# zju3dv/pvnet

Hardware: NVIDIA H100
Metric: images/sec (480x640, K=9) backbone+vote (higher is better)
Workload: dtype tf32 (fp32 storage, fp32 accumulate; vote fp32/fp64)

## Files before the change

pvnet_b200/csrc/conv_tc.cu:

```cuda
#include "conv_tc.cuh"
#include "ptx.cuh"

#include <cstdlib>
#include <mutex>
#include <new>

namespace pvnet {

struct ConvGeom {
    int Ho, Wo;
    int tiles_x, tiles_y, total_m_tiles;
    int TH, TW;
    int taps, cin_chunks, cin_pad;
    int Cout, BN;
    int out_cs, out_co;
    int res_cs, res_co;
    int act;
    int round_out;
    signed char tap_map[9];
    short tap_ox[9], tap_oy[9];
    int n_items;
    int stages;
};

struct AMaps {
    CUtensorMap m[4];
};

constexpr int CONV_THREADS = 288;
constexpr int CONV_KC = 32;
constexpr int CONV_A_BYTES = 128 * CONV_KC * 4;
constexpr int CONV_SLAB = 32;
constexpr int CONV_SLAB_BYTES = 128 * CONV_SLAB * 4;
constexpr int CONV_EPI_BAR = 1;

template <int BN, bool MC>
__global__ void __launch_bounds__(CONV_THREADS, 1)
    k_conv_tap(const __grid_constant__ AMaps amaps, const __grid_constant__ CUtensorMap tmB,
               const __grid_constant__ CUtensorMap tmOut, const __grid_constant__ CUtensorMap tmRes,
               const __grid_constant__ ConvGeom g, const float *__restrict__ bias, const int has_res)
{
    constexpr int B_BYTES = BN * CONV_KC * 4;
    constexpr int STAGE_BYTES = CONV_A_BYTES + B_BYTES;
    constexpr int SLABS = BN / CONV_SLAB;
    const int STAGES = g.stages;
    extern __shared__ uint8_t smem_raw[];
    uint8_t *smem = reinterpret_cast<uint8_t *>((reinterpret_cast<uintptr_t>(smem_raw) + 1023) & ~uintptr_t(1023));
    uint8_t *slab = smem + (size_t)STAGES * STAGE_BYTES;
    uint64_t *full = reinterpret_cast<uint64_t *>(slab + 2 * CONV_SLAB_BYTES);
    uint64_t *empty = full + STAGES;
    uint64_t *res_full = empty + STAGES;
    uint64_t *res_free = res_full + 2;

    const int warp = threadIdx.x >> 5, lane = threadIdx.x & 31;
    const int tiles_per_img = g.tiles_x * g.tiles_y;
    const int n_tiles_n = g.Cout / BN;
    const int nkb = g.taps * g.cin_chunks;
    const uint32_t crank = MC ? ptx::cluster_ctarank() : 0u;
    const int unit = MC ? (int)blockIdx.x >> 1 : (int)blockIdx.x, nunits = MC ? (int)gridDim.x >> 1 : (int)gridDim.x;
    auto item_tile = [&](int item, int &m_tile, int &n0) {
        const int mi = item / n_tiles_n;
        n0 = (item - mi * n_tiles_n) * BN;
        m_tile = MC ? min(2 * mi + (int)crank, g.total_m_tiles - 1) : mi;
    };

    if (threadIdx.x == 0) {
        for (int s = 0; s < STAGES; ++s) {
            ptx::mbar_init(&full[s], 1);
            ptx::mbar_init(&empty[s], MC ? 16 : 8);
        }
        for (int i = 0; i < 2; ++i) {
            ptx::mbar_init(&res_full[i], 1);
            ptx::mbar_init(&res_free[i], 1);
        }
        ptx::fence_barrier_init();
    }
    __syncthreads();
    if (MC) ptx::cluster_sync();

    if (warp == 8) {
        if (lane == 0) {
            int r_item = has_res ? unit : g.n_items, r_slab = 0;
            uint32_t rq = 0;
            auto poll_res = [&]() {
                if (r_item >= g.n_items) return;
                const uint32_t b = rq & 1u;
                if (!ptx::mbar_test_wait(&res_free[b], ((rq >> 1) & 1u) ^ 1u)) return;
                int m_tile, n0;
                item_tile(r_item, m_tile, n0);
                const int img = m_tile / tiles_per_img;
                const int trem = m_tile - img * tiles_per_img;
                const int tyi = trem / g.tiles_x, txi = trem - tyi * g.tiles_x;
                ptx::mbar_arrive_expect_tx(&res_full[b], (uint32_t)CONV_SLAB_BYTES);
                ptx::tma_load_4d(slab + b * CONV_SLAB_BYTES, &tmRes, &res_full[b], n0 + r_slab * CONV_SLAB, txi * g.TW,
                                 tyi * g.TH, img);
                ++rq;
                if (++r_slab == SLABS) {
                    r_slab = 0;
                    r_item += nunits;
                }
            };
            int s = 0;
            uint32_t ph = 0;
            for (int item = unit; item < g.n_items; item += nunits) {
                int m_tile, n0;
                item_tile(item, m_tile, n0);
                const int img = m_tile / tiles_per_img;
                const int trem = m_tile - img * tiles_per_img;
                const int tyi = trem / g.tiles_x, txi = trem - tyi * g.tiles_x;
                const int y0 = tyi * g.TH, x0 = txi * g.TW;
                for (int tap = 0; tap < g.taps; ++tap)
                    for (int cc = 0; cc < g.cin_chunks; ++cc) {
                        poll_res();
                        while (!(has_res ? ptx::mbar_test_wait(&empty[s], ph ^ 1u) : ptx::mbar_try_wait(&empty[s], ph ^ 1u)))
                            poll_res();
                        ptx::mbar_arrive_expect_tx(&full[s], (uint32_t)STAGE_BYTES);
                        uint8_t *sa = smem + (size_t)s * STAGE_BYTES;
                        ptx::tma_load_4d(sa, &amaps.m[g.tap_map[tap]], &full[s], cc * CONV_KC, x0 + g.tap_ox[tap],
                                         y0 + g.tap_oy[tap], img);
                        if (MC)
                            ptx::tma_load_2d_mc(sa + CONV_A_BYTES + crank * (B_BYTES / 2), &tmB, &full[s],
                                                tap * g.cin_pad + cc * CONV_KC, n0 + (int)crank * (BN / 2), (uint16_t)0x3);
                        else
                            ptx::tma_load_2d(sa + CONV_A_BYTES, &tmB, &full[s], tap * g.cin_pad + cc * CONV_KC, n0);
                        if (++s == STAGES) {
                            s = 0;
                            ph ^= 1u;
                        }
                    }
            }
            while (r_item < g.n_items) poll_res();
        }
    } else {
        const int wg = warp >> 2, wq = warp & 3;
        const int g8 = lane >> 2, t4 = lane & 3;
        const uint32_t smem_u = ptx::smem_u32(smem);
        auto release = [&](int st) {
            ptx::mbar_arrive(&empty[st]);
            if (MC) ptx::mbar_arrive_cluster(&empty[st], crank ^ 1u);
        };
        int s = 0;
        uint32_t ph = 0, sq = 0;
        for (int item = unit; item < g.n_items; item += nunits) {
            float acc[BN / 2];
#pragma unroll
            for (int i = 0; i < BN / 2; ++i) acc[i] = 0.f;
            int prev = -1;
            for (int kb = 0; kb < nkb; ++kb) {
                ptx::mbar_wait(&full[s], ph);
                const uint32_t sa = smem_u + (uint32_t)s * (uint32_t)STAGE_BYTES;
                const uint64_t adesc = ptx::make_kmajor_desc(sa + (uint32_t)(wg * 64 * 128), 128);
                const uint64_t bdesc = ptx::make_kmajor_desc(sa + (uint32_t)CONV_A_BYTES, 128);
                ptx::wgmma_fence();
#pragma unroll
                for (int k = 0; k < CONV_KC / 8; ++k)
                    ptx::Wgmma<BN>::ss(acc, adesc + (uint64_t)(2 * k), bdesc + (uint64_t)(2 * k), (kb | k) != 0 ? 1u : 0u);
                ptx::wgmma_commit();
                ptx::wgmma_wait<1>();
                ptx::fence_regs(acc);
                if (prev >= 0 && lane == 0) release(prev);
                prev = s;
                if (++s == STAGES) {
                    s = 0;
                    ph ^= 1u;
                }
            }
            ptx::wgmma_wait<0>();
            ptx::fence_regs(acc);
            if (lane == 0) release(prev);

            int m_tile, n0;
            item_tile(item, m_tile, n0);
            const int img = m_tile / tiles_per_img;
            const int trem = m_tile - img * tiles_per_img;
            const int tyi = trem / g.tiles_x, txi = trem - tyi * g.tiles_x;
            const uint32_t row_off = (uint32_t)((wg * 64 + wq * 16 + g8) * 128 + (t4 & 1) * 8);
            const uint32_t swz = (uint32_t)(((t4 >> 1) ^ g8) << 4);
            const uint32_t slab_u = ptx::smem_u32(slab);
#pragma unroll
            for (int j = 0; j < SLABS; ++j, ++sq) {
                const uint32_t b = sq & 1u;
                const uint32_t base = slab_u + b * (uint32_t)CONV_SLAB_BYTES + row_off;
                float2 bv[4];
#pragma unroll
                for (int jj = 0; jj < 4; ++jj)
                    bv[jj] = __ldg(reinterpret_cast<const float2 *>(bias + n0 + CONV_SLAB * j + 8 * jj + 2 * t4));
                if (has_res) ptx::mbar_wait(&res_full[b], (sq >> 1) & 1u);
                else ptx::named_bar_sync(CONV_EPI_BAR, 256);
#pragma unroll
                for (int jj = 0; jj < 4; ++jj)
#pragma unroll
                    for (int h = 0; h < 2; ++h) {
                        const uint32_t addr = base + (uint32_t)(h * 8 * 128) + (swz ^ (uint32_t)(32 * jj));
                        const int a = 4 * (4 * j + jj) + 2 * h;
                        float2 v = make_float2(acc[a] + bv[jj].x, acc[a + 1] + bv[jj].y);
                        if (has_res) {
                            const float2 r = ptx::lds64(addr);
                            v.x += r.x;
                            v.y += r.y;
                        }
                        v.x = epi_act(v.x, g.act, g.round_out);
                        v.y = epi_act(v.y, g.act, g.round_out);
                        ptx::sts64(addr, v);
                    }
                ptx::fence_proxy_async();
                ptx::named_bar_sync(CONV_EPI_BAR, 256);
                if (threadIdx.x == 0) {
                    ptx::tma_store_4d(&tmOut, slab + b * CONV_SLAB_BYTES, n0 + CONV_SLAB * j, txi * g.TW, tyi * g.TH, img);
                    ptx::tma_store_commit();
                    if (j == SLABS - 1) ptx::tma_store_wait_read();
                    else ptx::tma_store_wait_read1();
                    if (has_res) {
                        if (j > 0) ptx::mbar_arrive(&res_free[b ^ 1u]);
                        if (j == SLABS - 1) ptx::mbar_arrive(&res_free[b]);
                    }
                }
                __syncwarp();
            }
        }
        if (threadIdx.x == 0) ptx::tma_store_wait_all();
    }
    if (MC) ptx::cluster_sync();
}

typedef CUresult (*EncodeTiledFn)(CUtensorMap *, CUtensorMapDataType, cuuint32_t, void *, const cuuint64_t *,
                                  const cuuint64_t *, const cuuint32_t *, const cuuint32_t *, CUtensorMapInterleave,
                                  CUtensorMapSwizzle, CUtensorMapL2promotion, CUtensorMapFloatOOBfill);

static EncodeTiledFn encode_fn()
{
    static EncodeTiledFn fn = nullptr;
    static std::once_flag once;
    std::call_once(once, [] {
        void *p = nullptr;
        cudaDriverEntryPointQueryResult q;
        if (cudaGetDriverEntryPoint("cuTensorMapEncodeTiled", &p, cudaEnableDefault, &q) == cudaSuccess &&
            q == cudaDriverEntryPointSuccess)
            fn = reinterpret_cast<EncodeTiledFn>(p);
    });
    return fn;
}

int tma_encode(CUtensorMap *m, const void *base, int rank, const cuuint64_t *dims, const cuuint64_t *strides_bytes,
               const cuuint32_t *box, int swizzle_bytes)
{
    EncodeTiledFn fn = encode_fn();
    if (!fn) {
        set_error("cuTensorMapEncodeTiled entry point unavailable");
        return PVNET_E_CUDA;
    }
    cuuint32_t estr[5] = {1, 1, 1, 1, 1};
    const CUtensorMapSwizzle sw = swizzle_bytes == 128 ? CU_TENSOR_MAP_SWIZZLE_128B
                                  : swizzle_bytes == 64 ? CU_TENSOR_MAP_SWIZZLE_64B
                                                        : CU_TENSOR_MAP_SWIZZLE_32B;
    CUresult r = fn(m, CU_TENSOR_MAP_DATA_TYPE_FLOAT32, (cuuint32_t)rank, const_cast<void *>(base), dims,
                    strides_bytes, box, estr, CU_TENSOR_MAP_INTERLEAVE_NONE, sw, CU_TENSOR_MAP_L2_PROMOTION_L2_128B,
                    CU_TENSOR_MAP_FLOAT_OOB_FILL_NONE);
    if (r == CUDA_ERROR_INVALID_CONTEXT || r == CUDA_ERROR_NOT_INITIALIZED) {
        cudaFree(nullptr);
        r = fn(m, CU_TENSOR_MAP_DATA_TYPE_FLOAT32, (cuuint32_t)rank, const_cast<void *>(base), dims, strides_bytes, box, estr,
               CU_TENSOR_MAP_INTERLEAVE_NONE, sw, CU_TENSOR_MAP_L2_PROMOTION_L2_128B, CU_TENSOR_MAP_FLOAT_OOB_FILL_NONE);
    }
    if (r != CUDA_SUCCESS) {
        set_error("cuTensorMapEncodeTiled failed with CUresult %d (rank %d, dims %llu %llu, box %u %u, swizzle %d)",
                  (int)r, rank, (unsigned long long)dims[0], (unsigned long long)dims[1], box[0], box[1],
                  swizzle_bytes);
        return PVNET_E_CUDA;
    }
    return PVNET_OK;
}

struct ConvPlan {
    AMaps amaps;
    CUtensorMap tmB;
    CUtensorMap tmOut, tmRes;
    ConvGeom g;
    dim3 grid;
    size_t smem;
    int mc;
    const float *bias;
    int has_res;
};

int g_conv_persist = 1;
int g_conv_mc = 0;

int conv_plan(const ConvDesc &d, ConvPlan *p)
{
    PV_CHECK_ARG(d.in && d.w && d.bias && d.out, "conv: null pointer");
    PV_CHECK_ARG(!d.in2, "conv: a second input source is only supported by the column kernel");
    PV_CHECK_ARG(d.ksize == 1 || d.ksize == 3, "conv: kernel size %d unsupported", d.ksize);
    PV_CHECK_ARG(d.stride == 1 || d.stride == 2, "conv: stride %d unsupported", d.stride);
    PV_CHECK_ARG(d.stride == 1 || (d.dilation == 1 && d.H % 2 == 0 && d.W % 2 == 0),
                 "conv: stride 2 needs dilation 1 and even H,W");
    PV_CHECK_ARG(d.Cout % 32 == 0, "conv: Cout %d must be a multiple of 32", d.Cout);
    PV_CHECK_ARG(d.in_cs % 4 == 0 && d.in_co % 4 == 0 && d.out_cs % 4 == 0 && d.out_co % 4 == 0,
                 "conv: channel strides/offsets must be multiples of 4 floats");
    PV_CHECK_ARG(!d.res || (d.res_cs % 4 == 0 && d.res_co % 4 == 0), "conv: residual stride/offset alignment");
    PV_CHECK_ARG(((uintptr_t)d.in % 16 == 0) && ((uintptr_t)d.w % 16 == 0) && ((uintptr_t)d.out % 16 == 0) &&
                     ((uintptr_t)d.bias % 16 == 0),
                 "conv: pointers must be 16-byte aligned");
    PV_CHECK_ARG(d.Cin % 4 == 0, "conv: Cin %d must be a multiple of 4", d.Cin);
    const int kc = CONV_KC;
    ConvGeom &g = p->g;
    g.Ho = d.H / d.stride;
    g.Wo = d.W / d.stride;
    g.TH = 8;
    g.TW = 16;
    g.tiles_x = (g.Wo + g.TW - 1) / g.TW;
    g.tiles_y = (g.Ho + g.TH - 1) / g.TH;
    g.total_m_tiles = g.tiles_x * g.tiles_y * d.b;
    g.taps = d.ksize * d.ksize;
    g.cin_chunks = (d.Cin + kc - 1) / kc;
    g.cin_pad = g.cin_chunks * kc;
    g.Cout = d.Cout;
    {
        const long long sms = sm_count() > 0 ? sm_count() : 1;
        long long best = -1;
        for (int bn = 256; bn >= 32; bn >>= 1) {
            if (d.Cout % bn) continue;
            const long long items = (long long)g.total_m_tiles * (d.Cout / bn);
            const long long cost = (items + sms - 1) / sms * (CONV_A_BYTES + bn * kc * 4);
            if (best < 0 || cost < best) {
                best = cost;
                g.BN = bn;
            }
        }
    }
    g.out_cs = d.out_cs;
    g.out_co = d.out_co;
    g.res_cs = d.res_cs;
    g.res_co = d.res_co;
    g.act = d.act;
    g.round_out = d.round_out;
    const int pad = d.dilation * (d.ksize - 1) / 2;
    for (int t = 0; t < g.taps; ++t) {
        const int kh = t / d.ksize, kw = t - kh * d.ksize;
        if (d.stride == 1) {
            g.tap_map[t] = 0;
            g.tap_ox[t] = (short)(kw * d.dilation - pad);
            g.tap_oy[t] = (short)(kh * d.dilation - pad);
        } else {
            const int dy = kh - pad, dx = kw - pad;
            const int py = dy & 1, px = dx & 1;
            g.tap_map[t] = (signed char)(py * 2 + px);
            g.tap_oy[t] = (short)((dy - py) / 2);
            g.tap_ox[t] = (short)((dx - px) / 2);
        }
    }
    const int swz = kc * 4;
    const int nplanes = d.stride == 2 ? 4 : 1;
    for (int pl = 0; pl < nplanes; ++pl) {
        const int py = pl >> 1, px = pl & 1;
        const float *base = d.in + d.in_co + ((size_t)py * d.W + px) * d.in_cs;
        cuuint64_t dims[4] = {(cuuint64_t)d.Cin, (cuuint64_t)(d.W / d.stride), (cuuint64_t)(d.H / d.stride),
                              (cuuint64_t)d.b};
        cuuint64_t strides[3] = {(cuuint64_t)d.stride * d.in_cs * 4, (cuuint64_t)d.stride * d.W * d.in_cs * 4,
                                 (cuuint64_t)d.H * d.W * d.in_cs * 4};
        cuuint32_t box[4] = {(cuuint32_t)kc, (cuuint32_t)g.TW, (cuuint32_t)g.TH, 1};
        int rc = tma_encode(&p->amaps.m[pl], base, 4, dims, strides, box, swz);
        if (rc) return rc;
    }
    for (int pl = nplanes; pl < 4; ++pl) p->amaps.m[pl] = p->amaps.m[0];
    {
        cuuint64_t dims[2] = {(cuuint64_t)g.taps * g.cin_pad, (cuuint64_t)d.Cout};
        cuuint64_t strides[1] = {(cuuint64_t)g.taps * g.cin_pad * 4};
        p->mc = g_conv_mc;
        cuuint32_t box[2] = {(cuuint32_t)kc, (cuuint32_t)(p->mc ? g.BN / 2 : g.BN)};
        int rc = tma_encode(&p->tmB, d.w, 2, dims, strides, box, swz);
        if (rc) return rc;
    }
    {
        cuuint64_t dims[4] = {(cuuint64_t)d.Cout, (cuuint64_t)g.Wo, (cuuint64_t)g.Ho, (cuuint64_t)d.b};
        cuuint32_t box[4] = {(cuuint32_t)CONV_SLAB, (cuuint32_t)g.TW, (cuuint32_t)g.TH, 1};
        cuuint64_t ostr[3] = {(cuuint64_t)d.out_cs * 4, (cuuint64_t)g.Wo * d.out_cs * 4,
                              (cuuint64_t)g.Ho * g.Wo * d.out_cs * 4};
        int rc = tma_encode(&p->tmOut, d.out + d.out_co, 4, dims, ostr, box, CONV_SLAB * 4);
        if (rc) return rc;
        p->tmRes = p->tmOut;
        if (d.res) {
            PV_CHECK_ARG((uintptr_t)d.res % 16 == 0, "conv: pointers must be 16-byte aligned");
            cuuint64_t rstr[3] = {(cuuint64_t)d.res_cs * 4, (cuuint64_t)g.Wo * d.res_cs * 4,
                                  (cuuint64_t)g.Ho * g.Wo * d.res_cs * 4};
            rc = tma_encode(&p->tmRes, d.res + d.res_co, 4, dims, rstr, box, CONV_SLAB * 4);
            if (rc) return rc;
        }
    }
    const size_t stage_b = (size_t)CONV_A_BYTES + (size_t)g.BN * kc * 4;
    int st = (int)((227 * 1024 - 1024 - 256 - 2 * CONV_SLAB_BYTES) / stage_b);
    if (st > 8) st = 8;
    g.stages = st;
    p->smem = 1024 + (size_t)st * stage_b + 2 * CONV_SLAB_BYTES + 256;
    const int m_units = p->mc ? (g.total_m_tiles + 1) / 2 : g.total_m_tiles;
    g.n_items = m_units * (d.Cout / g.BN);
    long long units = g_conv_persist ? (long long)sm_count() / (p->mc ? 2 : 1) : (long long)g.n_items;
    if (units > g.n_items) units = g.n_items;
    p->grid = dim3((unsigned)(units * (p->mc ? 2 : 1)));
    p->bias = d.bias;
    p->has_res = d.res != nullptr;
    return PVNET_OK;
}

template <int BN, bool MC>
int conv_launch_t(const ConvPlan &p, cudaStream_t s)
{
    const cudaError_t attr_err = ensure_max_smem((const void *)k_conv_tap<BN, MC>, 227 * 1024);
    PV_CUDA(attr_err);
    cudaLaunchConfig_t cfg = {};
    cfg.gridDim = p.grid;
    cfg.blockDim = dim3(CONV_THREADS);
    cfg.dynamicSmemBytes = p.smem;
    cfg.stream = s;
    cudaLaunchAttribute attr[1];
    attr[0].id = cudaLaunchAttributeClusterDimension;
    attr[0].val.clusterDim.x = MC ? 2 : 1;
    attr[0].val.clusterDim.y = 1;
    attr[0].val.clusterDim.z = 1;
    cfg.attrs = attr;
    cfg.numAttrs = MC ? 1 : 0;
    PV_CUDA(cudaLaunchKernelEx(&cfg, k_conv_tap<BN, MC>, p.amaps, p.tmB, p.tmOut, p.tmRes, p.g, p.bias, p.has_res));
    PV_LAUNCHED("k_conv_tap");
    return PVNET_OK;
}

int conv_launch(const ConvPlan &p, cudaStream_t s)
{
    if (p.mc) {
        if (p.g.BN == 256) return conv_launch_t<256, true>(p, s);
        if (p.g.BN == 128) return conv_launch_t<128, true>(p, s);
        if (p.g.BN == 64) return conv_launch_t<64, true>(p, s);
        return conv_launch_t<32, true>(p, s);
    }
    if (p.g.BN == 256) return conv_launch_t<256, false>(p, s);
    if (p.g.BN == 128) return conv_launch_t<128, false>(p, s);
    if (p.g.BN == 64) return conv_launch_t<64, false>(p, s);
    return conv_launch_t<32, false>(p, s);
}

size_t conv_plan_size() { return sizeof(ConvPlan); }
int conv_plan_at(const ConvDesc &d, void *storage) { return conv_plan(d, new (storage) ConvPlan()); }
int conv_launch_at(const void *storage, cudaStream_t s) { return conv_launch(*static_cast<const ConvPlan *>(storage), s); }

}

extern "C" {

int pvnet_conv_set_multicast(int on)
{
    PV_CHECK_ARG(on == 0 || on == 1, "multicast mode must be 0 or 1");
    pvnet::g_conv_mc = on;
    return PVNET_OK;
}

int pvnet_conv_set_persistent(int on)
{
    pvnet::g_conv_persist = on ? 1 : 0;
    return PVNET_OK;
}

int pvnet_conv2d_nhwc(const float *in, int in_cs, int in_co, int Cin, const float *w_packed, const float *bias,
                      const float *res, int res_cs, int res_co, float *out, int out_cs, int out_co, int Cout, int b,
                      int H, int W, int ksize, int stride, int dilation, int act, int round_out,
                      pvnet_stream_t stream)
{
    pvnet::ConvDesc d{in, in_cs, in_co, Cin, w_packed, bias, res, res_cs, res_co, out, out_cs, out_co, Cout,
                      b, H, W, ksize, stride, dilation, act, round_out};
    const bool col = pvnet::g_conv_mode == 2 || (pvnet::g_conv_mode == 0 && pvnet::conv_col_eligible(d));
    if (col) {
        alignas(64) unsigned char storage[2048];
        static_assert(sizeof(storage) >= 1024, "plan storage");
        if (pvnet::conv_col_plan_size() > sizeof(storage)) {
            pvnet::set_error("column plan larger than its stack storage");
            return PVNET_E_STATE;
        }
        int rc = pvnet::conv_col_plan_at(d, nullptr, storage);
        if (rc) return rc;
        return pvnet::conv_col_launch_at(storage, (cudaStream_t)stream);
    }
    pvnet::ConvPlan plan;
    int rc = pvnet::conv_plan(d, &plan);
    if (rc) return rc;
    return pvnet::conv_launch(plan, (cudaStream_t)stream);
}

}
```

pvnet_b200/csrc/ptx.cuh:

```cuda
#pragma once
#include <cstdint>
#include <cuda.h>
#include <cuda_runtime.h>

namespace ptx {

__device__ __forceinline__ uint32_t smem_u32(const void *p)
{
    return static_cast<uint32_t>(__cvta_generic_to_shared(p));
}

__device__ __forceinline__ bool elect_one()
{
    uint32_t pred = 0;
    asm volatile(
        "{\n\t"
        ".reg .pred P1;\n\t"
        "elect.sync _|P1, 0xffffffff;\n\t"
        "selp.b32 %0, 1, 0, P1;\n\t"
        "}\n"
        : "=r"(pred));
    return pred != 0;
}

__device__ __forceinline__ void mbar_init(uint64_t *bar, uint32_t count)
{
    asm volatile("mbarrier.init.shared::cta.b64 [%0], %1;" ::"r"(smem_u32(bar)), "r"(count));
}
__device__ __forceinline__ void fence_barrier_init()
{
    asm volatile("fence.mbarrier_init.release.cluster;" ::: "memory");
}
__device__ __forceinline__ void fence_proxy_async()
{
    asm volatile("fence.proxy.async.shared::cta;" ::: "memory");
}
__device__ __forceinline__ void mbar_arrive_expect_tx(uint64_t *bar, uint32_t bytes)
{
    asm volatile("mbarrier.arrive.expect_tx.shared::cta.b64 _, [%0], %1;" ::"r"(smem_u32(bar)), "r"(bytes)
                 : "memory");
}
__device__ __forceinline__ void mbar_arrive(uint64_t *bar)
{
    asm volatile("mbarrier.arrive.shared::cta.b64 _, [%0];" ::"r"(smem_u32(bar)) : "memory");
}
__device__ __forceinline__ bool mbar_try_wait(uint64_t *bar, uint32_t parity)
{
    uint32_t ok;
    asm volatile(
        "{\n\t"
        ".reg .pred P1;\n\t"
        "mbarrier.try_wait.parity.shared::cta.b64 P1, [%1], %2;\n\t"
        "selp.b32 %0, 1, 0, P1;\n\t"
        "}\n"
        : "=r"(ok)
        : "r"(smem_u32(bar)), "r"(parity)
        : "memory");
    return ok != 0;
}
__device__ __forceinline__ bool mbar_test_wait(uint64_t *bar, uint32_t parity)
{
    uint32_t ok;
    asm volatile(
        "{\n\t"
        ".reg .pred P1;\n\t"
        "mbarrier.test_wait.parity.shared::cta.b64 P1, [%1], %2;\n\t"
        "selp.b32 %0, 1, 0, P1;\n\t"
        "}\n"
        : "=r"(ok)
        : "r"(smem_u32(bar)), "r"(parity)
        : "memory");
    return ok != 0;
}
__device__ __forceinline__ void mbar_wait(uint64_t *bar, uint32_t parity)
{
    while (!mbar_try_wait(bar, parity)) {
    }
}

__device__ __forceinline__ void prefetch_tensormap(const CUtensorMap *m)
{
    asm volatile("prefetch.tensormap [%0];" ::"l"(reinterpret_cast<uint64_t>(m)) : "memory");
}
__device__ __forceinline__ void tma_load_4d(void *smem_dst, const CUtensorMap *m, uint64_t *bar, int c0, int c1,
                                            int c2, int c3)
{
    asm volatile(
        "cp.async.bulk.tensor.4d.shared::cluster.global.mbarrier::complete_tx::bytes [%0], [%1, {%3, %4, %5, %6}], [%2];"
        ::"r"(smem_u32(smem_dst)), "l"(reinterpret_cast<uint64_t>(m)), "r"(smem_u32(bar)), "r"(c0), "r"(c1), "r"(c2),
        "r"(c3)
        : "memory");
}
__device__ __forceinline__ void tma_load_2d(void *smem_dst, const CUtensorMap *m, uint64_t *bar, int c0, int c1)
{
    asm volatile(
        "cp.async.bulk.tensor.2d.shared::cluster.global.mbarrier::complete_tx::bytes [%0], [%1, {%3, %4}], [%2];"
        ::"r"(smem_u32(smem_dst)), "l"(reinterpret_cast<uint64_t>(m)), "r"(smem_u32(bar)), "r"(c0), "r"(c1)
        : "memory");
}

__device__ __forceinline__ void tma_store_4d(const CUtensorMap *m, const void *smem_src, int c0, int c1, int c2, int c3)
{
    asm volatile("cp.async.bulk.tensor.4d.global.shared::cta.bulk_group [%0, {%2, %3, %4, %5}], [%1];" ::"l"(
                     reinterpret_cast<uint64_t>(m)),
                 "r"(smem_u32(smem_src)), "r"(c0), "r"(c1), "r"(c2), "r"(c3)
                 : "memory");
}
__device__ __forceinline__ void tma_store_commit() { asm volatile("cp.async.bulk.commit_group;" ::: "memory"); }
__device__ __forceinline__ void tma_store_wait_read() { asm volatile("cp.async.bulk.wait_group.read 0;" ::: "memory"); }
__device__ __forceinline__ void tma_store_wait_read1() { asm volatile("cp.async.bulk.wait_group.read 1;" ::: "memory"); }
__device__ __forceinline__ void tma_store_wait_all() { asm volatile("cp.async.bulk.wait_group 0;" ::: "memory"); }
__device__ __forceinline__ void sts128(uint32_t addr, float4 v)
{
    asm volatile("st.shared.v4.f32 [%0], {%1, %2, %3, %4};" ::"r"(addr), "f"(v.x), "f"(v.y), "f"(v.z), "f"(v.w) : "memory");
}
__device__ __forceinline__ float4 lds128(uint32_t addr)
{
    float4 v;
    asm volatile("ld.shared.v4.f32 {%0, %1, %2, %3}, [%4];" : "=f"(v.x), "=f"(v.y), "=f"(v.z), "=f"(v.w) : "r"(addr) : "memory");
    return v;
}
__device__ __forceinline__ void sts64(uint32_t addr, float2 v)
{
    asm volatile("st.shared.v2.f32 [%0], {%1, %2};" ::"r"(addr), "f"(v.x), "f"(v.y) : "memory");
}
__device__ __forceinline__ float2 lds64(uint32_t addr)
{
    float2 v;
    asm volatile("ld.shared.v2.f32 {%0, %1}, [%2];" : "=f"(v.x), "=f"(v.y) : "r"(addr) : "memory");
    return v;
}
__device__ __forceinline__ void sts32(uint32_t addr, float v) { asm volatile("st.shared.f32 [%0], %1;" ::"r"(addr), "f"(v) : "memory"); }
__device__ __forceinline__ float lds32(uint32_t addr)
{
    float v;
    asm volatile("ld.shared.f32 %0, [%1];" : "=f"(v) : "r"(addr) : "memory");
    return v;
}
__device__ __forceinline__ void sts8(uint32_t addr, uint32_t v) { asm volatile("st.shared.u8 [%0], %1;" ::"r"(addr), "r"(v) : "memory"); }
__device__ __forceinline__ uint32_t lds8(uint32_t addr)
{
    uint32_t v;
    asm volatile("ld.shared.u8 %0, [%1];" : "=r"(v) : "r"(addr) : "memory");
    return v;
}
__device__ __forceinline__ void tma_store_4d_u32(const CUtensorMap *m, uint32_t smem_src, int c0, int c1, int c2, int c3)
{
    asm volatile("cp.async.bulk.tensor.4d.global.shared::cta.bulk_group [%0, {%2, %3, %4, %5}], [%1];" ::"l"(
                     reinterpret_cast<uint64_t>(m)),
                 "r"(smem_src), "r"(c0), "r"(c1), "r"(c2), "r"(c3)
                 : "memory");
}
__device__ __forceinline__ void named_bar_sync(int id, int nthreads)
{
    asm volatile("bar.sync %0, %1;" ::"r"(id), "r"(nthreads) : "memory");
}

__device__ __forceinline__ uint32_t cluster_ctarank()
{
    uint32_t r;
    asm volatile("mov.u32 %0, %%cluster_ctarank;" : "=r"(r));
    return r;
}
__device__ __forceinline__ void cluster_sync()
{
    asm volatile("barrier.cluster.arrive.release.aligned;\n\tbarrier.cluster.wait.acquire.aligned;" ::: "memory");
}
__device__ __forceinline__ uint32_t mapa(const void *p, uint32_t rank)
{
    uint32_t r;
    asm volatile("mapa.shared::cluster.u32 %0, %1, %2;" : "=r"(r) : "r"(smem_u32(p)), "r"(rank));
    return r;
}
__device__ __forceinline__ float ld_cluster_f32(uint32_t addr)
{
    float v;
    asm volatile("ld.shared::cluster.f32 %0, [%1];" : "=f"(v) : "r"(addr) : "memory");
    return v;
}
__device__ __forceinline__ unsigned long long ld_cluster_u64(uint32_t addr)
{
    unsigned long long v;
    asm volatile("ld.shared::cluster.u64 %0, [%1];" : "=l"(v) : "r"(addr) : "memory");
    return v;
}
__device__ __forceinline__ void mbar_arrive_cluster(uint64_t *bar, uint32_t rank)
{
    asm volatile(
        "{\n\t.reg .b32 ra;\n\tmapa.shared::cluster.u32 ra, %0, %1;\n\t"
        "mbarrier.arrive.release.cluster.shared::cluster.b64 _, [ra];\n\t}" ::"r"(smem_u32(bar)), "r"(rank)
        : "memory");
}
__device__ __forceinline__ void tma_load_2d_mc(void *smem_dst, const CUtensorMap *m, uint64_t *bar, int c0, int c1,
                                               uint16_t cta_mask)
{
    asm volatile(
        "cp.async.bulk.tensor.2d.shared::cluster.global.mbarrier::complete_tx::bytes.multicast::cluster"
        " [%0], [%1, {%4, %5}], [%2], %3;"
        ::"r"(smem_u32(smem_dst)), "l"(reinterpret_cast<uint64_t>(m)), "r"(smem_u32(bar)), "h"(cta_mask), "r"(c0),
        "r"(c1)
        : "memory");
}

__device__ __forceinline__ void wgmma_fence() { asm volatile("wgmma.fence.sync.aligned;" ::: "memory"); }
__device__ __forceinline__ void wgmma_commit() { asm volatile("wgmma.commit_group.sync.aligned;" ::: "memory"); }
template <int N>
__device__ __forceinline__ void wgmma_wait() { asm volatile("wgmma.wait_group.sync.aligned %0;" ::"n"(N) : "memory"); }
template <int R>
__device__ __forceinline__ void fence_regs(float (&d)[R])
{
#pragma unroll
    for (int i = 0; i < R; ++i) asm volatile("" : "+f"(d[i])::"memory");
}

template <int N>
struct Wgmma;
template <>
struct Wgmma<32> {
    __device__ __forceinline__ static void ss(float (&d)[16], uint64_t adesc, uint64_t bdesc, uint32_t accumulate)
    {
        asm volatile(
            "{\n\t.reg .pred p;\n\tsetp.ne.b32 p, %18, 0;\n\t"
            "wgmma.mma_async.sync.aligned.m64n32k8.f32.tf32.tf32 {%0, %1, %2, %3, %4, %5, %6, %7, %8, %9, %10, %11, %12, %13, %14, %15}, %16, %17, p, 1, 1;\n\t}\n"
            : "+f"(d[0]), "+f"(d[1]), "+f"(d[2]), "+f"(d[3]), "+f"(d[4]), "+f"(d[5]), "+f"(d[6]), "+f"(d[7]), "+f"(d[8]), "+f"(d[9]), "+f"(d[10]), "+f"(d[11]), "+f"(d[12]), "+f"(d[13]), "+f"(d[14]), "+f"(d[15])
            : "l"(adesc), "l"(bdesc), "r"(accumulate));
    }
    __device__ __forceinline__ static void rs(float (&d)[16], const uint32_t (&a)[4], uint64_t bdesc, uint32_t accumulate)
    {
        asm volatile(
            "{\n\t.reg .pred p;\n\tsetp.ne.b32 p, %21, 0;\n\t"
            "wgmma.mma_async.sync.aligned.m64n32k8.f32.tf32.tf32 {%0, %1, %2, %3, %4, %5, %6, %7, %8, %9, %10, %11, %12, %13, %14, %15}, {%16, %17, %18, %19}, %20, p, 1, 1;\n\t}\n"
            : "+f"(d[0]), "+f"(d[1]), "+f"(d[2]), "+f"(d[3]), "+f"(d[4]), "+f"(d[5]), "+f"(d[6]), "+f"(d[7]), "+f"(d[8]), "+f"(d[9]), "+f"(d[10]), "+f"(d[11]), "+f"(d[12]), "+f"(d[13]), "+f"(d[14]), "+f"(d[15])
            : "r"(a[0]), "r"(a[1]), "r"(a[2]), "r"(a[3]), "l"(bdesc), "r"(accumulate));
    }
};

template <>
struct Wgmma<64> {
    __device__ __forceinline__ static void ss(float (&d)[32], uint64_t adesc, uint64_t bdesc, uint32_t accumulate)
    {
        asm volatile(
            "{\n\t.reg .pred p;\n\tsetp.ne.b32 p, %34, 0;\n\t"
            "wgmma.mma_async.sync.aligned.m64n64k8.f32.tf32.tf32 {%0, %1, %2, %3, %4, %5, %6, %7, %8, %9, %10, %11, %12, %13, %14, %15, %16, %17, %18, %19, %20, %21, %22, %23, %24, %25, %26, %27, %28, %29, %30, %31}, %32, %33, p, 1, 1;\n\t}\n"
            : "+f"(d[0]), "+f"(d[1]), "+f"(d[2]), "+f"(d[3]), "+f"(d[4]), "+f"(d[5]), "+f"(d[6]), "+f"(d[7]), "+f"(d[8]), "+f"(d[9]), "+f"(d[10]), "+f"(d[11]), "+f"(d[12]), "+f"(d[13]), "+f"(d[14]), "+f"(d[15]), "+f"(d[16]), "+f"(d[17]), "+f"(d[18]), "+f"(d[19]), "+f"(d[20]), "+f"(d[21]), "+f"(d[22]), "+f"(d[23]), "+f"(d[24]), "+f"(d[25]), "+f"(d[26]), "+f"(d[27]), "+f"(d[28]), "+f"(d[29]), "+f"(d[30]), "+f"(d[31])
            : "l"(adesc), "l"(bdesc), "r"(accumulate));
    }
    __device__ __forceinline__ static void rs(float (&d)[32], const uint32_t (&a)[4], uint64_t bdesc, uint32_t accumulate)
    {
        asm volatile(
            "{\n\t.reg .pred p;\n\tsetp.ne.b32 p, %37, 0;\n\t"
            "wgmma.mma_async.sync.aligned.m64n64k8.f32.tf32.tf32 {%0, %1, %2, %3, %4, %5, %6, %7, %8, %9, %10, %11, %12, %13, %14, %15, %16, %17, %18, %19, %20, %21, %22, %23, %24, %25, %26, %27, %28, %29, %30, %31}, {%32, %33, %34, %35}, %36, p, 1, 1;\n\t}\n"
            : "+f"(d[0]), "+f"(d[1]), "+f"(d[2]), "+f"(d[3]), "+f"(d[4]), "+f"(d[5]), "+f"(d[6]), "+f"(d[7]), "+f"(d[8]), "+f"(d[9]), "+f"(d[10]), "+f"(d[11]), "+f"(d[12]), "+f"(d[13]), "+f"(d[14]), "+f"(d[15]), "+f"(d[16]), "+f"(d[17]), "+f"(d[18]), "+f"(d[19]), "+f"(d[20]), "+f"(d[21]), "+f"(d[22]), "+f"(d[23]), "+f"(d[24]), "+f"(d[25]), "+f"(d[26]), "+f"(d[27]), "+f"(d[28]), "+f"(d[29]), "+f"(d[30]), "+f"(d[31])
            : "r"(a[0]), "r"(a[1]), "r"(a[2]), "r"(a[3]), "l"(bdesc), "r"(accumulate));
    }
};

template <>
struct Wgmma<128> {
    __device__ __forceinline__ static void ss(float (&d)[64], uint64_t adesc, uint64_t bdesc, uint32_t accumulate)
    {
        asm volatile(
            "{\n\t.reg .pred p;\n\tsetp.ne.b32 p, %66, 0;\n\t"
            "wgmma.mma_async.sync.aligned.m64n128k8.f32.tf32.tf32 {%0, %1, %2, %3, %4, %5, %6, %7, %8, %9, %10, %11, %12, %13, %14, %15, %16, %17, %18, %19, %20, %21, %22, %23, %24, %25, %26, %27, %28, %29, %30, %31, %32, %33, %34, %35, %36, %37, %38, %39, %40, %41, %42, %43, %44, %45, %46, %47, %48, %49, %50, %51, %52, %53, %54, %55, %56, %57, %58, %59, %60, %61, %62, %63}, %64, %65, p, 1, 1;\n\t}\n"
            : "+f"(d[0]), "+f"(d[1]), "+f"(d[2]), "+f"(d[3]), "+f"(d[4]), "+f"(d[5]), "+f"(d[6]), "+f"(d[7]), "+f"(d[8]), "+f"(d[9]), "+f"(d[10]), "+f"(d[11]), "+f"(d[12]), "+f"(d[13]), "+f"(d[14]), "+f"(d[15]), "+f"(d[16]), "+f"(d[17]), "+f"(d[18]), "+f"(d[19]), "+f"(d[20]), "+f"(d[21]), "+f"(d[22]), "+f"(d[23]), "+f"(d[24]), "+f"(d[25]), "+f"(d[26]), "+f"(d[27]), "+f"(d[28]), "+f"(d[29]), "+f"(d[30]), "+f"(d[31]), "+f"(d[32]), "+f"(d[33]), "+f"(d[34]), "+f"(d[35]), "+f"(d[36]), "+f"(d[37]), "+f"(d[38]), "+f"(d[39]), "+f"(d[40]), "+f"(d[41]), "+f"(d[42]), "+f"(d[43]), "+f"(d[44]), "+f"(d[45]), "+f"(d[46]), "+f"(d[47]), "+f"(d[48]), "+f"(d[49]), "+f"(d[50]), "+f"(d[51]), "+f"(d[52]), "+f"(d[53]), "+f"(d[54]), "+f"(d[55]), "+f"(d[56]), "+f"(d[57]), "+f"(d[58]), "+f"(d[59]), "+f"(d[60]), "+f"(d[61]), "+f"(d[62]), "+f"(d[63])
            : "l"(adesc), "l"(bdesc), "r"(accumulate));
    }
    __device__ __forceinline__ static void rs(float (&d)[64], const uint32_t (&a)[4], uint64_t bdesc, uint32_t accumulate)
    {
        asm volatile(
            "{\n\t.reg .pred p;\n\tsetp.ne.b32 p, %69, 0;\n\t"
            "wgmma.mma_async.sync.aligned.m64n128k8.f32.tf32.tf32 {%0, %1, %2, %3, %4, %5, %6, %7, %8, %9, %10, %11, %12, %13, %14, %15, %16, %17, %18, %19, %20, %21, %22, %23, %24, %25, %26, %27, %28, %29, %30, %31, %32, %33, %34, %35, %36, %37, %38, %39, %40, %41, %42, %43, %44, %45, %46, %47, %48, %49, %50, %51, %52, %53, %54, %55, %56, %57, %58, %59, %60, %61, %62, %63}, {%64, %65, %66, %67}, %68, p, 1, 1;\n\t}\n"
            : "+f"(d[0]), "+f"(d[1]), "+f"(d[2]), "+f"(d[3]), "+f"(d[4]), "+f"(d[5]), "+f"(d[6]), "+f"(d[7]), "+f"(d[8]), "+f"(d[9]), "+f"(d[10]), "+f"(d[11]), "+f"(d[12]), "+f"(d[13]), "+f"(d[14]), "+f"(d[15]), "+f"(d[16]), "+f"(d[17]), "+f"(d[18]), "+f"(d[19]), "+f"(d[20]), "+f"(d[21]), "+f"(d[22]), "+f"(d[23]), "+f"(d[24]), "+f"(d[25]), "+f"(d[26]), "+f"(d[27]), "+f"(d[28]), "+f"(d[29]), "+f"(d[30]), "+f"(d[31]), "+f"(d[32]), "+f"(d[33]), "+f"(d[34]), "+f"(d[35]), "+f"(d[36]), "+f"(d[37]), "+f"(d[38]), "+f"(d[39]), "+f"(d[40]), "+f"(d[41]), "+f"(d[42]), "+f"(d[43]), "+f"(d[44]), "+f"(d[45]), "+f"(d[46]), "+f"(d[47]), "+f"(d[48]), "+f"(d[49]), "+f"(d[50]), "+f"(d[51]), "+f"(d[52]), "+f"(d[53]), "+f"(d[54]), "+f"(d[55]), "+f"(d[56]), "+f"(d[57]), "+f"(d[58]), "+f"(d[59]), "+f"(d[60]), "+f"(d[61]), "+f"(d[62]), "+f"(d[63])
            : "r"(a[0]), "r"(a[1]), "r"(a[2]), "r"(a[3]), "l"(bdesc), "r"(accumulate));
    }
};

template <>
struct Wgmma<256> {
    __device__ __forceinline__ static void ss(float (&d)[128], uint64_t adesc, uint64_t bdesc, uint32_t accumulate)
    {
        asm volatile(
            "{\n\t.reg .pred p;\n\tsetp.ne.b32 p, %130, 0;\n\t"
            "wgmma.mma_async.sync.aligned.m64n256k8.f32.tf32.tf32 {%0, %1, %2, %3, %4, %5, %6, %7, %8, %9, %10, %11, %12, %13, %14, %15, %16, %17, %18, %19, %20, %21, %22, %23, %24, %25, %26, %27, %28, %29, %30, %31, %32, %33, %34, %35, %36, %37, %38, %39, %40, %41, %42, %43, %44, %45, %46, %47, %48, %49, %50, %51, %52, %53, %54, %55, %56, %57, %58, %59, %60, %61, %62, %63, %64, %65, %66, %67, %68, %69, %70, %71, %72, %73, %74, %75, %76, %77, %78, %79, %80, %81, %82, %83, %84, %85, %86, %87, %88, %89, %90, %91, %92, %93, %94, %95, %96, %97, %98, %99, %100, %101, %102, %103, %104, %105, %106, %107, %108, %109, %110, %111, %112, %113, %114, %115, %116, %117, %118, %119, %120, %121, %122, %123, %124, %125, %126, %127}, %128, %129, p, 1, 1;\n\t}\n"
            : "+f"(d[0]), "+f"(d[1]), "+f"(d[2]), "+f"(d[3]), "+f"(d[4]), "+f"(d[5]), "+f"(d[6]), "+f"(d[7]), "+f"(d[8]), "+f"(d[9]), "+f"(d[10]), "+f"(d[11]), "+f"(d[12]), "+f"(d[13]), "+f"(d[14]), "+f"(d[15]), "+f"(d[16]), "+f"(d[17]), "+f"(d[18]), "+f"(d[19]), "+f"(d[20]), "+f"(d[21]), "+f"(d[22]), "+f"(d[23]), "+f"(d[24]), "+f"(d[25]), "+f"(d[26]), "+f"(d[27]), "+f"(d[28]), "+f"(d[29]), "+f"(d[30]), "+f"(d[31]), "+f"(d[32]), "+f"(d[33]), "+f"(d[34]), "+f"(d[35]), "+f"(d[36]), "+f"(d[37]), "+f"(d[38]), "+f"(d[39]), "+f"(d[40]), "+f"(d[41]), "+f"(d[42]), "+f"(d[43]), "+f"(d[44]), "+f"(d[45]), "+f"(d[46]), "+f"(d[47]), "+f"(d[48]), "+f"(d[49]), "+f"(d[50]), "+f"(d[51]), "+f"(d[52]), "+f"(d[53]), "+f"(d[54]), "+f"(d[55]), "+f"(d[56]), "+f"(d[57]), "+f"(d[58]), "+f"(d[59]), "+f"(d[60]), "+f"(d[61]), "+f"(d[62]), "+f"(d[63]), "+f"(d[64]), "+f"(d[65]), "+f"(d[66]), "+f"(d[67]), "+f"(d[68]), "+f"(d[69]), "+f"(d[70]), "+f"(d[71]), "+f"(d[72]), "+f"(d[73]), "+f"(d[74]), "+f"(d[75]), "+f"(d[76]), "+f"(d[77]), "+f"(d[78]), "+f"(d[79]), "+f"(d[80]), "+f"(d[81]), "+f"(d[82]), "+f"(d[83]), "+f"(d[84]), "+f"(d[85]), "+f"(d[86]), "+f"(d[87]), "+f"(d[88]), "+f"(d[89]), "+f"(d[90]), "+f"(d[91]), "+f"(d[92]), "+f"(d[93]), "+f"(d[94]), "+f"(d[95]), "+f"(d[96]), "+f"(d[97]), "+f"(d[98]), "+f"(d[99]), "+f"(d[100]), "+f"(d[101]), "+f"(d[102]), "+f"(d[103]), "+f"(d[104]), "+f"(d[105]), "+f"(d[106]), "+f"(d[107]), "+f"(d[108]), "+f"(d[109]), "+f"(d[110]), "+f"(d[111]), "+f"(d[112]), "+f"(d[113]), "+f"(d[114]), "+f"(d[115]), "+f"(d[116]), "+f"(d[117]), "+f"(d[118]), "+f"(d[119]), "+f"(d[120]), "+f"(d[121]), "+f"(d[122]), "+f"(d[123]), "+f"(d[124]), "+f"(d[125]), "+f"(d[126]), "+f"(d[127])
            : "l"(adesc), "l"(bdesc), "r"(accumulate));
    }
};

__device__ __forceinline__ float round_tf32(float x)
{
    uint32_t r;
    asm("cvt.rna.tf32.f32 %0, %1;" : "=r"(r) : "f"(x));
    return __uint_as_float(r);
}


__device__ __forceinline__ uint64_t make_kmajor_desc(uint32_t smem_addr, uint32_t swizzle_bytes)
{
    const uint64_t layout = swizzle_bytes == 128 ? 1ull : (swizzle_bytes == 64 ? 2ull : 3ull);
    const uint64_t sbo = (8ull * swizzle_bytes) >> 4;
    return (uint64_t)((smem_addr & 0x3ffff) >> 4) | (1ull << 16) | (sbo << 32) | (layout << 62);
}
__device__ __forceinline__ uint64_t make_kmajor_desc(uint32_t smem_addr, uint32_t swizzle_bytes, uint32_t sbo_bytes)
{
    const uint64_t layout = swizzle_bytes == 128 ? 1ull : (swizzle_bytes == 64 ? 2ull : 3ull);
    return (uint64_t)((smem_addr & 0x3ffff) >> 4) | (1ull << 16) | ((uint64_t)(sbo_bytes >> 4) << 32) | (layout << 62);
}
__device__ __forceinline__ uint32_t swizzle_off(uint32_t off, uint32_t swizzle_bytes)
{
    return off ^ ((off >> 3) & (swizzle_bytes - 16u));
}

}
```

Baseline: 1723.

## Load residual tiles through main pipeline stages instead of separate polled slab ring

Residual tiles are now loaded by the producer warp into the regular operand pipeline stages after each item's K-loop, reusing the full/empty mbarriers. This replaces the separate two-slab residual ring that was polled with test_wait inside the main load loop. The epilogue reads the residual from the stage buffer and releases the stage afterwards. It also skips duplicate TMA stores for clamped multicast tiles and relaxes the store-wait to allow one store in flight. The cost is that residual loads now occupy pipeline stages, which may delay prefetch of the next item's operands, and the epilogue now always takes a named barrier sync.

Measured after the change: 1752, median of 6. 1.02x the previous value.

```diff
diff --git a/pvnet_b200/csrc/conv_tc.cu b/pvnet_b200/csrc/conv_tc.cu
--- a/pvnet_b200/csrc/conv_tc.cu
+++ b/pvnet_b200/csrc/conv_tc.cu
@@ -43,14 +43,14 @@
     constexpr int B_BYTES = BN * CONV_KC * 4;
     constexpr int STAGE_BYTES = CONV_A_BYTES + B_BYTES;
     constexpr int SLABS = BN / CONV_SLAB;
+    constexpr int RES_PER_STAGE = STAGE_BYTES / CONV_SLAB_BYTES;
+    constexpr int RES_STAGES = (SLABS + RES_PER_STAGE - 1) / RES_PER_STAGE;
     const int STAGES = g.stages;
     extern __shared__ uint8_t smem_raw[];
     uint8_t *smem = reinterpret_cast<uint8_t *>((reinterpret_cast<uintptr_t>(smem_raw) + 1023) & ~uintptr_t(1023));
     uint8_t *slab = smem + (size_t)STAGES * STAGE_BYTES;
     uint64_t *full = reinterpret_cast<uint64_t *>(slab + 2 * CONV_SLAB_BYTES);
     uint64_t *empty = full + STAGES;
-    uint64_t *res_full = empty + STAGES;
-    uint64_t *res_free = res_full + 2;
 
     const int warp = threadIdx.x >> 5, lane = threadIdx.x & 31;
     const int tiles_per_img = g.tiles_x * g.tiles_y;
@@ -69,10 +69,6 @@
             ptx::mbar_init(&full[s], 1);
             ptx::mbar_init(&empty[s], MC ? 16 : 8);
         }
-        for (int i = 0; i < 2; ++i) {
-            ptx::mbar_init(&res_full[i], 1);
-            ptx::mbar_init(&res_free[i], 1);
-        }
         ptx::fence_barrier_init();
     }
     __syncthreads();
@@ -80,26 +76,6 @@
 
     if (warp == 8) {
         if (lane == 0) {
-            int r_item = has_res ? unit : g.n_items, r_slab = 0;
-            uint32_t rq = 0;
-            auto poll_res = [&]() {
-                if (r_item >= g.n_items) return;
-                const uint32_t b = rq & 1u;
-                if (!ptx::mbar_test_wait(&res_free[b], ((rq >> 1) & 1u) ^ 1u)) return;
-                int m_tile, n0;
-                item_tile(r_item, m_tile, n0);
-                const int img = m_tile / tiles_per_img;
-                const int trem = m_tile - img * tiles_per_img;
-                const int tyi = trem / g.tiles_x, txi = trem - tyi * g.tiles_x;
-                ptx::mbar_arrive_expect_tx(&res_full[b], (uint32_t)CONV_SLAB_BYTES);
-                ptx::tma_load_4d(slab + b * CONV_SLAB_BYTES, &tmRes, &res_full[b], n0 + r_slab * CONV_SLAB, txi * g.TW,
-                                 tyi * g.TH, img);
-                ++rq;
-                if (++r_slab == SLABS) {
-                    r_slab = 0;
-                    r_item += nunits;
-                }
-            };
             int s = 0;
             uint32_t ph = 0;
             for (int item = unit; item < g.n_items; item += nunits) {
@@ -111,9 +87,7 @@
                 const int y0 = tyi * g.TH, x0 = txi * g.TW;
                 for (int tap = 0; tap < g.taps; ++tap)
                     for (int cc = 0; cc < g.cin_chunks; ++cc) {
-                        poll_res();
-                        while (!(has_res ? ptx::mbar_test_wait(&empty[s], ph ^ 1u) : ptx::mbar_try_wait(&empty[s], ph ^ 1u)))
-                            poll_res();
+                        ptx::mbar_wait(&empty[s], ph ^ 1u);
                         ptx::mbar_arrive_expect_tx(&full[s], (uint32_t)STAGE_BYTES);
                         uint8_t *sa = smem + (size_t)s * STAGE_BYTES;
                         ptx::tma_load_4d(sa, &amaps.m[g.tap_map[tap]], &full[s], cc * CONV_KC, x0 + g.tap_ox[tap],
@@ -128,8 +102,22 @@
                             ph ^= 1u;
                         }
                     }
+                if (has_res)
+#pragma unroll
+                    for (int r = 0; r < RES_STAGES; ++r) {
+                        const int n = min(RES_PER_STAGE, SLABS - r * RES_PER_STAGE);
+                        ptx::mbar_wait(&empty[s], ph ^ 1u);
+                        ptx::mbar_arrive_expect_tx(&full[s], (uint32_t)(n * CONV_SLAB_BYTES));
+                        uint8_t *sr = smem + (size_t)s * STAGE_BYTES;
+                        for (int k = 0; k < n; ++k)
+                            ptx::tma_load_4d(sr + k * CONV_SLAB_BYTES, &tmRes, &full[s],
+                                             n0 + (r * RES_PER_STAGE + k) * CONV_SLAB, x0, y0, img);
+                        if (++s == STAGES) {
+                            s = 0;
+                            ph ^= 1u;
+                        }
+                    }
             }
-            while (r_item < g.n_items) poll_res();
         }
     } else {
         const int wg = warp >> 2, wq = warp & 3;
@@ -171,6 +159,7 @@
 
             int m_tile, n0;
             item_tile(item, m_tile, n0);
+            const bool stores = !MC || m_tile == 2 * (item / n_tiles_n) + (int)crank;
             const int img = m_tile / tiles_per_img;
             const int trem = m_tile - img * tiles_per_img;
             const int tyi = trem / g.tiles_x, txi = trem - tyi * g.tiles_x;
@@ -179,41 +168,49 @@
             const uint32_t slab_u = ptx::smem_u32(slab);
 #pragma unroll
             for (int j = 0; j < SLABS; ++j, ++sq) {
+                const int k = j % RES_PER_STAGE;
                 const uint32_t b = sq & 1u;
                 const uint32_t base = slab_u + b * (uint32_t)CONV_SLAB_BYTES + row_off;
+                const uint32_t rbase = smem_u + (uint32_t)s * (uint32_t)STAGE_BYTES + (uint32_t)(k * CONV_SLAB_BYTES) + row_off;
                 float2 bv[4];
 #pragma unroll
                 for (int jj = 0; jj < 4; ++jj)
                     bv[jj] = __ldg(reinterpret_cast<const float2 *>(bias + n0 + CONV_SLAB * j + 8 * jj + 2 * t4));
-                if (has_res) ptx::mbar_wait(&res_full[b], (sq >> 1) & 1u);
-                else ptx::named_bar_sync(CONV_EPI_BAR, 256);
+                if (has_res && k == 0) ptx::mbar_wait(&full[s], ph);
+                ptx::named_bar_sync(CONV_EPI_BAR, 256);
 #pragma unroll
                 for (int jj = 0; jj < 4; ++jj)
 #pragma unroll
                     for (int h = 0; h < 2; ++h) {
-                        const uint32_t addr = base + (uint32_t)(h * 8 * 128) + (swz ^ (uint32_t)(32 * jj));
+                        const uint32_t off = (uint32_t)(h * 8 * 128) + (swz ^ (uint32_t)(32 * jj));
                         const int a = 4 * (4 * j + jj) + 2 * h;
                         float2 v = make_float2(acc[a] + bv[jj].x, acc[a + 1] + bv[jj].y);
                         if (has_res) {
-                            const float2 r = ptx::lds64(addr);
+                            const float2 r = ptx::lds64(rbase + off);
                             v.x += r.x;
                             v.y += r.y;
                         }
                         v.x = epi_act(v.x, g.act, g.round_out);
                         v.y = epi_act(v.y, g.act, g.round_out);
-                        ptx::sts64(addr, v);
+                        ptx::sts64(base + off, v);
                     }
+                if (has_res && (k == RES_PER_STAGE - 1 || j == SLABS - 1)) {
+                    __syncwarp();
+                    if (lane == 0) release(s);
+                    if (++s == STAGES) {
+                        s = 0;
+                        ph ^= 1u;
+                    }
+                }
                 ptx::fence_proxy_async();
                 ptx::named_bar_sync(CONV_EPI_BAR, 256);
                 if (threadIdx.x == 0) {
-                    ptx::tma_store_4d(&tmOut, slab + b * CONV_SLAB_BYTES, n0 + CONV_SLAB * j, txi * g.TW, tyi * g.TH, img);
-                    ptx::tma_store_commit();
-                    if (j == SLABS - 1) ptx::tma_store_wait_read();
-                    else ptx::tma_store_wait_read1();
-                    if (has_res) {
-                        if (j > 0) ptx::mbar_arrive(&res_free[b ^ 1u]);
-                        if (j == SLABS - 1) ptx::mbar_arrive(&res_free[b]);
+                    if (stores) {
+                        ptx::tma_store_4d(&tmOut, slab + b * CONV_SLAB_BYTES, n0 + CONV_SLAB * j, txi * g.TW, tyi * g.TH,
+                                          img);
+                        ptx::tma_store_commit();
                     }
+                    ptx::tma_store_wait_read1();
                 }
                 __syncwarp();
             }
diff --git a/pvnet_b200/csrc/ptx.cuh b/pvnet_b200/csrc/ptx.cuh
--- a/pvnet_b200/csrc/ptx.cuh
+++ b/pvnet_b200/csrc/ptx.cuh
@@ -58,20 +58,6 @@
         : "memory");
     return ok != 0;
 }
-__device__ __forceinline__ bool mbar_test_wait(uint64_t *bar, uint32_t parity)
-{
-    uint32_t ok;
-    asm volatile(
-        "{\n\t"
-        ".reg .pred P1;\n\t"
-        "mbarrier.test_wait.parity.shared::cta.b64 P1, [%1], %2;\n\t"
-        "selp.b32 %0, 1, 0, P1;\n\t"
-        "}\n"
-        : "=r"(ok)
-        : "r"(smem_u32(bar)), "r"(parity)
-        : "memory");
-    return ok != 0;
-}
 __device__ __forceinline__ void mbar_wait(uint64_t *bar, uint32_t parity)
 {
     while (!mbar_try_wait(bar, parity)) {
```
